# tensorlayer/HyperPose

Hardware: AMD Instinct MI355X
Metric: end-to-end FPS (preproc+DNN+PAF parse) @ 368x432 (higher is better)
Workload: dtype f32; 1 GPU; configs[1]: Lightweight-OpenPose (MobilenetDilated) + PAF parser, batch 8 @ 368x432 per GPU; frames from pinned host memory (one H2D per batch), parser on the network's own maps, humans to the host; key=configs[1]/f32, global_batch=8, parallelism=frame-sharded x1, no steady-state collective, pipes_per_gpu=4, parser_input=the network's own heat-maps

## Files before the change

### hyperpose_amd/csrc/conv_fp32.hip

```cpp
#include "conv_fp32.hpp"

#include "conv32_epilogue.hpp"
#include "conv_device.hpp"

#include <algorithm>
#include <cstdlib>

namespace hp {

namespace {

typedef float f32x4 __attribute__((ext_vector_type(4)));

__device__ __forceinline__ float act32(float v, int act, float param, float alpha)
{
    switch (act) {
    case ACT_RELU:
        return fmaxf(v, 0.f);
    case ACT_RELU6:
        return fminf(fmaxf(v, 0.f), 6.f);
    case ACT_LEAKY:
        return v > 0.f ? v : v * param;
    case ACT_PRELU:
        return v > 0.f ? v : v * alpha;
    case ACT_SIGMOID:
        return 1.f / (1.f + expf(-v));
    case ACT_SOFTPLUS:
        return v > 20.f ? v : log1pf(expf(v));
    default:
        return v;
    }
}

__device__ __forceinline__ long tv32_off(const tview32& t, int b, int y, int x)
{
    return ((long)b * t.img + (long)y * t.wp + x) * t.cs + t.coff;
}

}

template <int BM, int BN, int WM, int WN, bool ROWS>
__global__ __launch_bounds__(256) void conv32_kernel(const conv32_params p)
{
    constexpr int BK = 16, LDR = 20;
    constexpr int TM = BM / WM / 32, TN = BN / WN / 32, NA = BM / 64, NB = BN / 64;
    static_assert(WM * WN == 4 && TM >= 1 && TN >= 1 && NA >= 1 && NB >= 1, "tile");
    constexpr int AB_BYTES = 2 * (BM + BN) * LDR * 4, SLABS = 4 * rows_geom<TM>::SLAB_BYTES;
    __shared__ __attribute__((aligned(16))) unsigned char lds_raw[AB_BYTES > SLABS ? AB_BYTES : SLABS];
    float (*const sA)[BM * LDR] = reinterpret_cast<float (*)[BM * LDR]>(lds_raw);
    float (*const sB)[BN * LDR] = reinterpret_cast<float (*)[BN * LDR]>(lds_raw + 2 * BM * LDR * 4);

    const int tid = threadIdx.x, lane = tid & 63, wave = tid >> 6;
    const int wm = wave / WN, wn = wave % WN;
    const int G = p.Cout_pad / BM, nx = (p.npix + BN - 1) / BN;
    const int bj = blockIdx.x >> 3, ptile = (bj / G) * 8 + (blockIdx.x & 7);
    if (ptile >= nx)
        return;
    const int n0 = ptile * BN, m0 = (bj % G) * BM;
    const int lrow = tid >> 2, lchunk = (tid & 3) * 4;
    const int OHW = p.OH * p.OW, kc = p.Cin / BK, steps = p.KH * p.KW * kc;

    long bbase[NB];
#pragma unroll
    for (int j = 0; j < NB; ++j) {
        const int n = min(n0 + lrow + 64 * j, p.npix - 1);
        const int b = n / OHW, rem = n - b * OHW;
        const int oy = rem / p.OW, ox = rem - oy * p.OW;
        bbase[j] = tv32_off(p.in, b, oy * p.stride - p.pad_t, ox * p.stride - p.pad_l) + lchunk;
    }
    const float* const wrow = p.w + (long)(m0 + lrow) * p.Cin + lchunk;

    f32x4 ra[NA], rb[NB];
    auto gload = [&](int s) {
        const int tap = s / kc, k0 = (s - tap * kc) * BK;
        const int ky = tap / p.KW, kx = tap - ky * p.KW;
        const long toff = ((long)(ky * p.dil) * p.in.wp + kx * p.dil) * p.in.cs + k0;
        const float* const wt = wrow + (long)tap * p.Cout_pad * p.Cin + k0;
#pragma unroll
        for (int j = 0; j < NA; ++j)
            ra[j] = *reinterpret_cast<const f32x4*>(wt + (long)(64 * j) * p.Cin);
#pragma unroll
        for (int j = 0; j < NB; ++j)
            rb[j] = *reinterpret_cast<const f32x4*>(p.in.p + bbase[j] + toff);
    };
    auto to_lds = [&](int buf) {
#pragma unroll
        for (int j = 0; j < NA; ++j)
            *reinterpret_cast<f32x4*>(&sA[buf][(lrow + 64 * j) * LDR + lchunk]) = ra[j];
#pragma unroll
        for (int j = 0; j < NB; ++j)
            *reinterpret_cast<f32x4*>(&sB[buf][(lrow + 64 * j) * LDR + lchunk]) = rb[j];
    };

    floatx16 acc[TM][TN];
#pragma unroll
    for (int i = 0; i < TM; ++i)
#pragma unroll
        for (int j = 0; j < TN; ++j)
#pragma unroll
            for (int r = 0; r < 16; ++r)
                acc[i][j][r] = 0.f;

    const int frow = lane & 31, fh = (lane >> 5) * 4;
    int dbg_i = 0;
#define HP_STAMP()                                       \
    if (p.dbg && blockIdx.x == 9 && tid == 0)            \
        p.dbg[dbg_i++] = __builtin_amdgcn_s_memtime();
    HP_STAMP();
    if (p.dbg && tid == 0 && blockIdx.x < 4096) {
        p.dbg[128 + 3 * blockIdx.x] = __builtin_amdgcn_s_memrealtime();
        p.dbg[128 + 3 * blockIdx.x + 2] = ((unsigned long long)__builtin_amdgcn_s_getreg((31 << 11) | 20) << 32) | (unsigned)__builtin_amdgcn_s_getreg((31 << 11) | 4);
    }
    gload(0);
    to_lds(0);
    lds_barrier();
    HP_STAMP();
#pragma unroll 1
    for (int s = 0; s < steps; ++s) {
        gload(min(s + 1, steps - 1));
        const float* const a_s = &sA[s & 1][(wm * TM * 32 + frow) * LDR + fh];
        const float* const b_s = &sB[s & 1][(wn * TN * 32 + frow) * LDR + fh];
#pragma unroll
        for (int kk = 0; kk < BK / 8; ++kk) {
            f32x4 fa[TM], fb[TN];
#pragma unroll
            for (int i = 0; i < TM; ++i)
                fa[i] = *reinterpret_cast<const f32x4*>(a_s + i * 32 * LDR + kk * 8);
#pragma unroll
            for (int j = 0; j < TN; ++j)
                fb[j] = *reinterpret_cast<const f32x4*>(b_s + j * 32 * LDR + kk * 8);
#pragma unroll
            for (int e = 0; e < 4; ++e)
#pragma unroll
                for (int i = 0; i < TM; ++i)
#pragma unroll
                    for (int j = 0; j < TN; ++j)
                        acc[i][j] = __builtin_amdgcn_mfma_f32_32x32x2f32(fa[i][e], fb[j][e], acc[i][j], 0, 0, 0);
        }
        to_lds((s + 1) & 1);
        lds_barrier();
        if ((s & 7) == 7)
            HP_STAMP();
    }

    if constexpr (ROWS) {
        lds_barrier();
        float* const slab = reinterpret_cast<float*>(lds_raw) + wave * (rows_geom<TM>::SLAB_BYTES / 4);
#pragma unroll
        for (int j = 0; j < TN; ++j) {
            floatx16 fin[TM];
#pragma unroll
            for (int i = 0; i < TM; ++i)
                fin[i] = acc[i][j];
            const int nb = n0 + (wn * TN + j) * 32;
            conv32_store_rows<TM>(p, fin, slab, lane, m0 + wm * TM * 32, [&](int r, bool& ok, long& ooff, long& roff) {
                const int n = nb + r;
                ok = n < p.npix;
                const int nc = min(n, p.npix - 1);
                const int b = nc / OHW, rem = nc - b * OHW;
                const int oy = rem / p.OW, ox = rem - oy * p.OW;
                ooff = tv32_off(p.out, b, oy, ox);
                roff = p.res.p ? tv32_off(p.res, b, oy, ox) : 0;
            });
        }
    } else {
    const bool out_vec = p.out.p && ((p.out.coff | p.out.cs) & 3) == 0;
    const bool res_vec = p.res.p && ((p.res.coff | p.res.cs) & 3) == 0;
    const bool res_pre = p.res.p && p.res_before_act, res_post = p.res.p && !p.res_before_act;
#pragma unroll
    for (int j = 0; j < TN; ++j) {
        const int n = n0 + (wn * TN + j) * 32 + frow;
        const bool pix_ok = n < p.npix;
        const int nc = min(n, p.npix - 1);
        const int b = nc / OHW, rem = nc - b * OHW;
        const int oy = rem / p.OW, ox = rem - oy * p.OW;
        const long ooff = p.out.p ? tv32_off(p.out, b, oy, ox) : 0;
        const long roff = p.res.p ? tv32_off(p.res, b, oy, ox) : 0;
#pragma unroll
        for (int i = 0; i < TM; ++i) {
#pragma unroll
            for (int q = 0; q < 4; ++q) {
                const int m = m0 + (wm * TM + i) * 32 + 8 * q + fh;
                if (pix_ok && m < p.Cout) {
                    const bool full = m + 3 < p.Cout;
                    float v[4], rr[4] = { 0.f, 0.f, 0.f, 0.f };
                    if (p.res.p) {
                        if (full && res_vec) {
                            const f32x4 t = *reinterpret_cast<const f32x4*>(p.res.p + roff + m);
                            rr[0] = t[0], rr[1] = t[1], rr[2] = t[2], rr[3] = t[3];
                        } else {
#pragma unroll
                            for (int e = 0; e < 4; ++e)
                                if (m + e < p.Cout)
                                    rr[e] = p.res.p[roff + m + e];
                        }
                    }
                    const f32x4 bs = *reinterpret_cast<const f32x4*>(p.bias + m);
                    f32x4 sl = { p.act_slope, p.act_slope, p.act_slope, p.act_slope };
                    if (p.alpha)
                        sl = *reinterpret_cast<const f32x4*>(p.alpha + m);
#pragma unroll
                    for (int e = 0; e < 4; ++e) {
                        float x = acc[i][j][4 * q + e] + bs[e];
                        if (res_pre)
                            x += rr[e];
                        x = x > 0.f ? fminf(x, p.act_hi) : x * sl[e];
                        if (res_post)
                            x += rr[e];
                        v[e] = x;
                    }
                    if (p.out.p) {
                        if (full && out_vec) {
                            f32x4 t = { v[0], v[1], v[2], v[3] };
                            *reinterpret_cast<f32x4*>(p.out.p + ooff + m) = t;
                        } else {
#pragma unroll
                            for (int e = 0; e < 4; ++e)
                                if (m + e < p.Cout)
                                    p.out.p[ooff + m + e] = v[e];
                        }
                    }
                    if (p.out_f32) {
#pragma unroll
                        for (int e = 0; e < 4; ++e)
                            if (m + e < p.Cout)
                                p.out_f32[((long)b * p.Cout + m + e) * OHW + rem] = v[e];
                    }
                }
            }
        }
    }
    }
    HP_STAMP();
    if (p.dbg && tid == 0 && blockIdx.x < 4096)
        p.dbg[128 + 3 * blockIdx.x + 1] = __builtin_amdgcn_s_memrealtime();
#undef HP_STAMP
}

template <int BN, int WN = 2>
__global__ __launch_bounds__(256) void conv32_t16_kernel(const conv32_params p)
{
    constexpr int BM = 64, BK = 16, WM = 4 / WN, TMW = BM / 16 / WM, TNW = BN / WN / 16;
    constexpr int NB = (BN + 63) / 64, BR = NB * 64;
    static_assert(BN % (16 * WN) == 0 && (WN == 1 || WN == 2), "wavefront columns of whole 16-pixel tiles");
    __shared__ __attribute__((aligned(16))) float lds[2 * (BM + BR) * BK];
    float (*const sA)[BM * BK] = reinterpret_cast<float (*)[BM * BK]>(lds);
    float (*const sB)[BR * BK] = reinterpret_cast<float (*)[BR * BK]>(lds + 2 * BM * BK);

    const int tid = threadIdx.x, lane = tid & 63, wave = tid >> 6;
    const int wm = WN == 2 ? wave >> 1 : wave, wn = WN == 2 ? wave & 1 : 0;
    const int G = p.Cout_pad / BM, nx = (p.npix + BN - 1) / BN;
    const int bj = blockIdx.x >> 3, ptile = (bj / G) * 8 + (blockIdx.x & 7);
    if (ptile >= nx)
        return;
    const int n0 = ptile * BN, m0 = (bj % G) * BM;
    const int lrow = tid >> 2, lq = tid & 3;
    const int OHW = p.OH * p.OW, kc = p.Cin / BK, steps = p.KH * p.KW * kc;
    auto swz = [](int row, int quad) { return row * BK + ((quad ^ (((row >> 3) & 1) << 1)) << 2); };

    long bbase[NB];
#pragma unroll
    for (int j = 0; j < NB; ++j) {
        const int n = min(n0 + min(lrow + 64 * j, BN - 1), p.npix - 1);
        const int b = n / OHW, rem = n - b * OHW;
        const int oy = rem / p.OW, ox = rem - oy * p.OW;
        bbase[j] = tv32_off(p.in, b, oy * p.stride - p.pad_t, ox * p.stride - p.pad_l) + lq * 4;
    }
    const float* const wrow = p.w + (long)(m0 + lrow) * p.Cin + lq * 4;
    f32x4 ra, rb[NB];
    auto gload = [&](int s) {
        const int tap = s / kc, k0 = (s - tap * kc) * BK;
        const int ky = tap / p.KW, kx = tap - ky * p.KW;
        const long toff = ((long)(ky * p.dil) * p.in.wp + kx * p.dil) * p.in.cs + k0;
        ra = *reinterpret_cast<const f32x4*>(wrow + (long)tap * p.Cout_pad * p.Cin + k0);
#pragma unroll
        for (int j = 0; j < NB; ++j)
            rb[j] = *reinterpret_cast<const f32x4*>(p.in.p + bbase[j] + toff);
    };
    auto to_lds = [&](int buf) {
        *reinterpret_cast<f32x4*>(&sA[buf][swz(lrow, lq)]) = ra;
#pragma unroll
        for (int j = 0; j < NB; ++j)
            *reinterpret_cast<f32x4*>(&sB[buf][swz(lrow + 64 * j, lq)]) = rb[j];
    };

    f32x4 acc[TMW][TNW];
#pragma unroll
    for (int i = 0; i < TMW; ++i)
#pragma unroll
        for (int j = 0; j < TNW; ++j)
            acc[i][j] = f32x4{ 0.f, 0.f, 0.f, 0.f };

    const int fr = lane & 15, kq = lane >> 4;
    int dbg_i = 0;
#define HP_STAMP()                                       \
    if (p.dbg && blockIdx.x == 9 && tid == 0)            \
        p.dbg[dbg_i++] = __builtin_amdgcn_s_memtime();
    HP_STAMP();
    if (p.dbg && tid == 0 && blockIdx.x < 4096) {
        p.dbg[128 + 3 * blockIdx.x] = __builtin_amdgcn_s_memrealtime();
        p.dbg[128 + 3 * blockIdx.x + 2] = ((unsigned long long)__builtin_amdgcn_s_getreg((31 << 11) | 20) << 32) | (unsigned)__builtin_amdgcn_s_getreg((31 << 11) | 4);
    }
    gload(0);
    to_lds(0);
    lds_barrier();
    HP_STAMP();
#pragma unroll 1
    for (int s = 0; s < steps; ++s) {
        gload(min(s + 1, steps - 1));
        f32x4 fa[TMW], fb[TNW];
#pragma unroll
        for (int i = 0; i < TMW; ++i)
            fa[i] = *reinterpret_cast<const f32x4*>(&sA[s & 1][swz(wm * (16 * TMW) + i * 16 + fr, kq)]);
#pragma unroll
        for (int j = 0; j < TNW; ++j)
            fb[j] = *reinterpret_cast<const f32x4*>(&sB[s & 1][swz(wn * (BN / WN) + j * 16 + fr, kq)]);
#pragma unroll
        for (int e = 0; e < 4; ++e)
#pragma unroll
            for (int i = 0; i < TMW; ++i)
#pragma unroll
                for (int j = 0; j < TNW; ++j)
                    acc[i][j] = __builtin_amdgcn_mfma_f32_16x16x4f32(fa[i][e], fb[j][e], acc[i][j], 0, 0, 0);
        to_lds((s + 1) & 1);
        lds_barrier();
        if ((s & 7) == 7)
            HP_STAMP();
    }

    const int q = lane >> 4;
    const bool out_vec = p.out.p && ((p.out.coff | p.out.cs) & 3) == 0;
    const bool res_vec = p.res.p && ((p.res.coff | p.res.cs) & 3) == 0;
    const bool res_pre = p.res.p && p.res_before_act, res_post = p.res.p && !p.res_before_act;
    f32x4 bs[TMW], sl[TMW];
#pragma unroll
    for (int i = 0; i < TMW; ++i) {
        const int m = m0 + wm * (16 * TMW) + i * 16 + 4 * q;
        bs[i] = *reinterpret_cast<const f32x4*>(p.bias + m);
        sl[i] = f32x4{ p.act_slope, p.act_slope, p.act_slope, p.act_slope };
        if (p.alpha)
            sl[i] = *reinterpret_cast<const f32x4*>(p.alpha + m);
    }
#pragma unroll
    for (int j = 0; j < TNW; ++j) {
        const int n = n0 + wn * (BN / WN) + j * 16 + fr;
        const bool pix_ok = n < p.npix;
        const int nc = min(n, p.npix - 1);
        const int b = nc / OHW, rem = nc - b * OHW;
        const int oy = rem / p.OW, ox = rem - oy * p.OW;
        const long ooff = p.out.p ? tv32_off(p.out, b, oy, ox) : 0;
        const long roff = p.res.p ? tv32_off(p.res, b, oy, ox) : 0;
#pragma unroll
        for (int i = 0; i < TMW; ++i) {
            const int m = m0 + wm * (16 * TMW) + i * 16 + 4 * q;
            if (!pix_ok || m >= p.Cout)
                continue;
            const bool full = m + 3 < p.Cout;
            float v[4], rr[4] = { 0.f, 0.f, 0.f, 0.f };
            if (p.res.p) {
                if (full && res_vec) {
                    const f32x4 t = *reinterpret_cast<const f32x4*>(p.res.p + roff + m);
                    rr[0] = t[0], rr[1] = t[1], rr[2] = t[2], rr[3] = t[3];
                } else {
#pragma unroll
                    for (int e = 0; e < 4; ++e)
                        if (m + e < p.Cout)
                            rr[e] = p.res.p[roff + m + e];
                }
            }
#pragma unroll
            for (int e = 0; e < 4; ++e) {
                float x = acc[i][j][e] + bs[i][e];
                if (res_pre)
                    x += rr[e];
                x = x > 0.f ? fminf(x, p.act_hi) : x * sl[i][e];
                if (res_post)
                    x += rr[e];
                v[e] = x;
            }
            if (p.out.p) {
                if (full && out_vec)
                    *reinterpret_cast<f32x4*>(p.out.p + ooff + m) = f32x4{ v[0], v[1], v[2], v[3] };
                else {
#pragma unroll
                    for (int e = 0; e < 4; ++e)
                        if (m + e < p.Cout)
                            p.out.p[ooff + m + e] = v[e];
                }
            }
// ... 131 lines not shown
                const long ooff = s_out[prow] + m;
                float v[4], rv[4] = { 0.f, 0.f, 0.f, 0.f };
                if (p.res.p) {
                    if (res_vec) {
                        rv[0] = rr[j][h][r][0], rv[1] = rr[j][h][r][1], rv[2] = rr[j][h][r][2], rv[3] = rr[j][h][r][3];
                    } else {
                        const long roff = s_res[prow] + m;
#pragma unroll
                        for (int e = 0; e < 4; ++e)
                            if (m + e < p.Cout)
                                rv[e] = p.res.p[roff + e];
                    }
                }
#pragma unroll
                for (int e = 0; e < 4; ++e) {
                    float x = a[e] + bsr[h][e];
                    if (res_pre)
                        x += rv[e];
                    x = x > 0.f ? fminf(x, p.act_hi) : x * slr[h][e];
                    if (res_post)
                        x += rv[e];
                    v[e] = x;
                }
                if (full && out_vec)
                    *reinterpret_cast<f32x4*>(p.out.p + ooff) = f32x4{ v[0], v[1], v[2], v[3] };
                else {
#pragma unroll
                    for (int e = 0; e < 4; ++e)
                        if (m + e < p.Cout)
                            p.out.p[ooff + e] = v[e];
                }
            }
            __builtin_amdgcn_wave_barrier();
        }
    }
}

template <int KT, int BN>
static hipError_t launch_wk(const conv32_params& p, dim3 grid, hipStream_t s)
{
    constexpr int lds = KT / 16 * ((64 * 16 + 16) + (BN * 16 + 16)) * 4 + 4 * 16 * 36 * 4 + 3 * BN * 8;
    static bool granted = false;
    if (lds > 64 * 1024 && !granted) {
        const hipError_t e = hipFuncSetAttribute((const void*)conv32_wk_kernel<KT, BN>, hipFuncAttributeMaxDynamicSharedMemorySize, lds);
        if (e != hipSuccess)
            return e;
        granted = true;
    }
    HP_LAUNCH((conv32_wk_kernel<KT, BN>), grid, dim3(256), lds, s, p);
    return hipGetLastError();
}

static int conv32_wk_bn(const conv32_params& p, const engine_switches& sw)
{
    const int wk = sw.c32_wk;
    if (wk == 0 || p.KH != 1 || p.KW != 1 || p.dil != 1 || p.out_f32 || !p.out.p || (p.Cin != 32 && p.Cin != 64 && p.Cin != 128))
        return 0;
    if (p.Cin == 128 && wk != 1)
        return 0;
    const int bn = 64;
    const long np = p.pick_npix > 0 ? p.pick_npix : p.npix, blocks = (np + bn - 1) / bn * (p.Cout_pad / 64);
    return wk == 1 || blocks >= 768 ? bn : 0;
}

static void conv32_pick(const conv32_params& p, const engine_switches& sw, int& BM, int& BN)
{
    BM = p.Cout_pad % 128 == 0 ? 128 : 64, BN = 128;
    const long blocks = (long)(((p.pick_npix > 0 ? p.pick_npix : p.npix) + 127) / 128) * (p.Cout_pad / BM);
    if (blocks < 448)
        BM = 64, BN = 64;
    else if (blocks < 1024 && BM == 128)
        BM = 64;
    const int bn160 = sw.c32_bn160;
    if (bn160 == 1 || bn160 == 176) {
        BM = 64, BN = bn160 == 1 ? 160 : 176;
        return;
    }
    if (BM == 64 && BN == 128 && bn160 != 0) {
        const long np = p.pick_npix > 0 ? p.pick_npix : p.npix;
        const long g = p.Cout_pad / 64, b128 = (long)((np + 127) / 128) * g, b160 = (long)((np + 159) / 160) * g;
        if (b128 > 1024 && b160 <= 1024)
            BN = 160;
    }
    if (bn160 != 0 && p.KH == 1 && p.KW == 1 && p.stride == 1 && p.Cin <= 128 && p.Cout_pad >= 256 && !p.out_f32 && (BN == 128))
        BM = 64, BN = 160;
}

static bool conv32_rows(const conv32_params& p, int BN)
{
    if (BN == 160 || BN == 176)
        return false;
    return !p.out_f32 && (p.lane_epilogue < 0 || (p.lane_epilogue == 0 && BN == 64));
}

int conv32_tile(const conv32_params& p, const engine_switches& sw)
{
    if (const int bn = conv32_wk_bn(p, sw))
        return 39000000 + p.Cin * 1000 + bn;
    int BM, BN;
    conv32_pick(p, sw, BM, BN);
    return 32000000 + (conv32_rows(p, BN) ? 400000 : 0) + BM * 1000 + BN;
}

bool set_act32(conv32_params& p)
{
    const float inf = __builtin_huge_valf();
    switch (p.act) {
    case ACT_NONE:
        p.act_slope = 1.f, p.act_hi = inf;
        return true;
    case ACT_RELU:
        p.act_slope = 0.f, p.act_hi = inf;
        return true;
    case ACT_RELU6:
        p.act_slope = 0.f, p.act_hi = 6.f;
        return true;
    case ACT_LEAKY:
        p.act_slope = p.act_param, p.act_hi = inf;
        return true;
    case ACT_PRELU:
        p.act_slope = 0.f, p.act_hi = inf;
        return p.alpha != nullptr;
    default:
        return false;
    }
}

hipError_t launch_conv32(const conv32_params& p, const engine_switches& sw, hipStream_t s)
{
    if (p.Cin % 16 || p.Cout_pad % 64 || p.npix <= 0)
        return hipErrorInvalidValue;
    if (const int bn = conv32_wk_bn(p, sw)) {
        const dim3 g(((p.npix + bn - 1) / bn + 7) / 8 * 8 * (p.Cout_pad / 64));
        return p.Cin == 32 ? launch_wk<32, 64>(p, g, s) : p.Cin == 64 ? launch_wk<64, 64>(p, g, s) : launch_wk<128, 64>(p, g, s);
    }
    int BM, BN;
    conv32_pick(p, sw, BM, BN);
    const dim3 grid(((p.npix + BN - 1) / BN + 7) / 8 * 8 * (p.Cout_pad / BM));
    const bool rows = conv32_rows(p, BN);
#define HP_C32_CASE(BM_, BN_, WM_, WN_)                                                    \
    if (rows)                                                                              \
        HP_LAUNCH((conv32_kernel<BM_, BN_, WM_, WN_, true>), grid, dim3(256), 0, s, p);    \
    else                                                                                   \
        HP_LAUNCH((conv32_kernel<BM_, BN_, WM_, WN_, false>), grid, dim3(256), 0, s, p);
    if (BN == 176) {
        HP_LAUNCH((conv32_t16_kernel<176, 1>), grid, dim3(256), 0, s, p);
    } else if (BN == 160) {
        HP_LAUNCH((conv32_t16_kernel<160>), grid, dim3(256), 0, s, p);
    } else if (BM == 128) {
        HP_C32_CASE(128, 128, 2, 2)
    } else if (BN == 128) {
        HP_C32_CASE(64, 128, 1, 4)
    } else {
        HP_C32_CASE(64, 64, 2, 2)
    }
#undef HP_C32_CASE
    return hipGetLastError();
}

__device__ unsigned g_first_conv_verify[4];
__global__ __launch_bounds__(256) void first_conv32_kernel(const first_conv32_params p, int tiles_x, int tiles_y, int TH, int GP, int verify)
{
    extern __shared__ __attribute__((aligned(16))) float s_w32[];
    constexpr int TW = 8, PX = 4;
    const int G = (p.Cout + 7) / 8, CP = G * 8, taps = p.KH * p.KW;
    const int IH = (TH - 1) * p.stride + p.KH, IW = (TW - 1) * p.stride + p.KW;
    float* const s_x = s_w32 + taps * 3 * CP;
    int t = blockIdx.x;
    const int tx = t % tiles_x;
    t /= tiles_x;
    const int ty = t % tiles_y, b = t / tiles_y;
    const int oy0 = ty * TH, ox0 = tx * TW;
    const int iy0 = oy0 * p.stride - p.pad_t, ix0 = ox0 * p.stride - p.pad_l;
    for (int i = threadIdx.x; i < taps * 3 * CP; i += 256) {
        const int co = i % CP, tc = i / CP;
        s_w32[i] = co < p.Cout ? p.w[(size_t)co * taps * 3 + tc] : 0.f;
    }
    for (int i = threadIdx.x; i < IH * IW; i += 256) {
        const int py = i / IW, px = i - py * IW;
        const int iy = iy0 + py, ix = ix0 + px;
        float v[3] = { 0.f, 0.f, 0.f };
        if (iy >= 0 && iy < p.H && ix >= 0 && ix < p.W) {
            if (p.in_u8) {
                const uint8_t* q = p.in_u8 + (((size_t)b * p.H + iy) * p.W + ix) * 3;
#pragma unroll
                for (int c = 0; c < 3; ++c)
                    v[c] = ((float)((double)q[p.flip_rb ? 2 - c : c] * p.factor) - p.mean[c]) * p.inv_std[c];
            } else {
#pragma unroll
                for (int c = 0; c < 3; ++c)
                    v[c] = (p.in_f32[(((size_t)b * 3 + c) * p.H + iy) * p.W + ix] - p.mean[c]) * p.inv_std[c];
            }
        }
        s_x[i * 3] = v[0], s_x[i * 3 + 1] = v[1], s_x[i * 3 + 2] = v[2];
    }
    __syncthreads();
    const int g0 = threadIdx.x % GP, slot = threadIdx.x / GP;
    auto verify_lds = [&]() {
        if (!verify)
            return;
        unsigned bad_x = 0, bad_w = 0;
        for (int i = threadIdx.x; i < IH * IW; i += 256) {
            const int py = i / IW, px = i - py * IW;
            const int iy = iy0 + py, ix = ix0 + px;
            float v[3] = { 0.f, 0.f, 0.f };
            if (iy >= 0 && iy < p.H && ix >= 0 && ix < p.W && p.in_u8) {
                const uint8_t* q = p.in_u8 + (((size_t)b * p.H + iy) * p.W + ix) * 3;
                for (int c = 0; c < 3; ++c)
                    v[c] = ((float)((double)q[p.flip_rb ? 2 - c : c] * p.factor) - p.mean[c]) * p.inv_std[c];
            }
            for (int c = 0; c < 3; ++c)
                bad_x += __float_as_uint(s_x[i * 3 + c]) != __float_as_uint(v[c]);
        }
        for (int i = threadIdx.x; i < taps * 3 * CP; i += 256) {
            const int co = i % CP, tc = i / CP;
            const float wv = co < p.Cout ? p.w[(size_t)co * taps * 3 + tc] : 0.f;
            bad_w += __float_as_uint(s_w32[i]) != __float_as_uint(wv);
        }
        if (bad_x)
            atomicAdd(&g_first_conv_verify[0], bad_x);
        if (bad_w)
            atomicAdd(&g_first_conv_verify[1], bad_w);
        if (threadIdx.x == 0)
            atomicAdd(&g_first_conv_verify[2], 1u);
    };
    if (slot >= TH * (TW / PX)) {
        verify_lds();
        return;
    }
    const int ly = slot / (TW / PX), lx0 = (slot % (TW / PX)) * PX;
    const int oy = oy0 + ly;
    if (oy >= p.OH) {
        verify_lds();
        return;
    }
    const bool vec_ok = ((p.out.coff | p.out.cs) & 3) == 0;
    for (int g = g0; g < G; g += GP) {
        float acc[PX][8];
#pragma unroll
        for (int r = 0; r < 8; ++r) {
            const float bv = (g * 8 + r < p.Cout) ? p.bias[g * 8 + r] : 0.f;
#pragma unroll
            for (int j = 0; j < PX; ++j)
                acc[j][r] = bv;
        }
        for (int ky = 0; ky < p.KH; ++ky)
            for (int kx = 0; kx < p.KW; ++kx) {
                const float* xp = s_x + ((ly * p.stride + ky) * IW + lx0 * p.stride + kx) * 3;
                const float* wt = s_w32 + (size_t)((ky * p.KW + kx) * 3) * CP + g * 8;
#pragma unroll
                for (int c = 0; c < 3; ++c) {
                    const f32x4 w0 = *reinterpret_cast<const f32x4*>(wt + c * CP);
                    const f32x4 w1 = *reinterpret_cast<const f32x4*>(wt + c * CP + 4);
#pragma unroll
                    for (int j = 0; j < PX; ++j) {
                        const float xv = xp[j * p.stride * 3 + c];
#pragma unroll
                        for (int e = 0; e < 4; ++e)
                            acc[j][e] = fmaf(xv, w0[e], acc[j][e]), acc[j][4 + e] = fmaf(xv, w1[e], acc[j][4 + e]);
                    }
                }
            }
        if (verify) {
            float acc2[PX][8];
#pragma unroll
            for (int r = 0; r < 8; ++r) {
                const float bv = (g * 8 + r < p.Cout) ? p.bias[g * 8 + r] : 0.f;
#pragma unroll
                for (int j = 0; j < PX; ++j)
                    acc2[j][r] = bv;
            }
            for (int ky = 0; ky < p.KH; ++ky)
                for (int kx = 0; kx < p.KW; ++kx) {
                    const float* xp = s_x + ((ly * p.stride + ky) * IW + lx0 * p.stride + kx) * 3;
                    const float* wt = s_w32 + (size_t)((ky * p.KW + kx) * 3) * CP + g * 8;
#pragma unroll
                    for (int c = 0; c < 3; ++c) {
                        const f32x4 w0 = *reinterpret_cast<const f32x4*>(wt + c * CP);
                        const f32x4 w1 = *reinterpret_cast<const f32x4*>(wt + c * CP + 4);
#pragma unroll
                        for (int j = 0; j < PX; ++j) {
                            const float xv = xp[j * p.stride * 3 + c];
#pragma unroll
                            for (int e = 0; e < 4; ++e)
                                acc2[j][e] = fmaf(xv, w0[e], acc2[j][e]), acc2[j][4 + e] = fmaf(xv, w1[e], acc2[j][4 + e]);
                        }
                    }
                }
            unsigned bad = 0;
#pragma unroll
            for (int j = 0; j < PX; ++j)
#pragma unroll
                for (int r = 0; r < 8; ++r)
                    bad += __float_as_uint(acc[j][r]) != __float_as_uint(acc2[j][r]);
            if (bad)
                atomicAdd(&g_first_conv_verify[3], bad);
        }
#pragma unroll
        for (int j = 0; j < PX; ++j) {
            const int ox = ox0 + lx0 + j;
            if (ox >= p.OW)
                break;
            float* op = p.out.p + tv32_off(p.out, b, oy, ox) + g * 8;
            if (g * 8 + 7 < p.Cout && vec_ok) {
                f32x4 o0, o1;
#pragma unroll
                for (int e = 0; e < 4; ++e)
// ... 293 lines not shown
```

### hyperpose_amd/csrc/engine.cpp

```cpp
#include "conv_fp32.hpp"
#include "conv_i8.hpp"
#include "conv_kernels.hpp"
#include "engine_timeline.hpp"
#include "hp_common.hpp"
#include "weight_pack.hpp"

#include <algorithm>
#include <cmath>
#include <map>
#include <memory>
#include <string>
#include <variant>
#include <cstdio>
#include <cstdlib>
#include <vector>

namespace {

inline int round_up(int a, int b) { return (a + b - 1) / b * b; }

struct tensor_info {
    bool defined = false;
    bool elided = false;
    bool unwritten = false;
// ... 1654 lines not shown
{
    hd = hp::timeline_header{};
    hd.layer = st.layer;
    switch (st.kind) {
    case launch_kind::conv16: {
        const auto& c = std::get<conv16_launch>(b);
        if (c.i8 || !switches.dbg_conv || hp::conv_mfma_tile(c.cp) / 100000 != 52)
            return false;
        kind = hp::timeline_kind::conv, hd.cin = c.cp.Cin, hd.cout = c.cp.Cout, hd.tile = hp::conv_mfma_tile(c.cp);
        return true;
    }
    case launch_kind::bneck:
        kind = hp::timeline_kind::bneck, hd.tile = hp::bottleneck_variant(std::get<hp::bneck_params>(b));
        return switches.dbg_bn;
    case launch_kind::chain:
        kind = hp::timeline_kind::chain, hd.tile = hp::conv_chain_variant(std::get<hp::chain_params>(b));
        return switches.dbg_chain;
    case launch_kind::sep:
        kind = hp::timeline_kind::sep, hd.cin = std::get<hp::sep_params>(b).C;
        return switches.dbg_sep;
    case launch_kind::conv32:
    case launch_kind::wino2:
    case launch_kind::wino3:
    case launch_kind::direct: {
        const hp::conv32_params& q = std::get<conv32_launch>(b).cp;
        if (!switches.dbg_direct || (st.kind == launch_kind::conv32 && q.Cin < switches.dbg_min_cin))
            return false;
        kind = st.kind == launch_kind::conv32 ? hp::timeline_kind::conv32
            : st.kind == launch_kind::wino2   ? hp::timeline_kind::wino
            : st.kind == launch_kind::wino3   ? hp::timeline_kind::wino3
                                              : hp::timeline_kind::direct;
        hd.cin = q.Cin, hd.cout = q.Cout, hd.kh = q.KH, hd.kw = q.KW, hd.tile = tile_of(st.kind, b);
        if (st.kind == launch_kind::wino2)
            (void)hp::conv32_winograd_occupancy(q, &hd.blocks_per_cu);
        return true;
    }
    default: return false;
    }
}

int hp_engine::trace_step(const step& st, launch_payload& b, hipStream_t s) const
{
    hp::timeline_kind kind;
    hp::timeline_header hd;
    if (!timeline_of(st, b, kind, hd))
        return HP_OK;
    const size_t words = hp::timeline_words(kind);
    hp::dev_buf buf;
    HP_TRY(buf.alloc(words * 8));
    HP_HIP_TRY(hipMemset(buf.p, 0, words * 8));
    HP_TRY(launch(st.kind, b, s, buf.as<unsigned long long>()));
    HP_HIP_TRY(hipStreamSynchronize(s));
    std::vector<unsigned long long> hv(words);
    HP_HIP_TRY(hipMemcpy(hv.data(), buf.p, words * 8, hipMemcpyDeviceToHost));
    hp::print_timeline(stderr, kind, hd, hv.data());
    return HP_OK;
}

int hp_engine::run_step(const step& st, const uint8_t* u8, const float* f32, int n, hipStream_t s, int b0) const
{
    launch_payload b = bound(st, u8, f32, n, b0);
    HP_TRY(launch(st.kind, b, s, nullptr));
    return trace_step(st, b, s);
}

int hp_engine::launch_head_pair32(size_t i, int n, int b0, hipStream_t s, bool* done) const
{
    *done = false;
    if (i + 1 >= steps.size() || steps[i].kind != launch_kind::head32 || steps[i + 1].kind != launch_kind::head32)
        return HP_OK;
    const auto &ha = steps[i].as<head32_launch>(), &hb = steps[i + 1].as<head32_launch>();
    const hp::conv32_params a = bind(ha.cp, n, b0), b = bind(hb.cp, n, b0);
    if (!hp::conv32_head_pair_ok(a, b, switches))
        return HP_OK;
    HP_HIP_TRY(hp::launch_conv32_head_pair(a, ha.hh, b, hb.hh, s));
    *done = true;
    return HP_OK;
}

int hp_engine::enqueue_range(const uint8_t* u8, const float* f32, int b0, int n, hipStream_t s) const
{
    for (size_t i = 0; i < steps.size(); ++i) {
        bool paired = false;
        HP_TRY(launch_head_pair32(i, n, b0, s, &paired));
        if (paired)
            ++i;
        else
            HP_TRY(run_step(steps[i], u8, f32, n, s, b0));
    }
    for (auto& o : outputs)
        if (o.fused_layer < 0) {
            const tensor_info& ti = *tensors[o.tensor];
            float* const dst = o.buf->as<float>() + (size_t)b0 * o.out_c() * o.x.out_h * o.x.out_w;
            if (is_f32())
                HP_HIP_TRY(hp::launch_output_transform32(at_frame(ti.view32(o.coff), b0), n, o.H, o.W, o.x, dst, s));
            else
                HP_HIP_TRY(hp::launch_output_transform(ti.view(o.coff), n, o.H, o.W, o.x, dst, s));
        }
    return HP_OK;
}

void hp_engine::fill_row(hp_layer_time* out, int k, int cap, const step& st, int n, float ms) const
{
    if (!out || k >= cap)
        return;
    out[k].layer = st.layer, out[k].op = st.op;
    out[k].tile = step_tile(st, n);
    out[k].ms = ms;
    out[k].flops = st.flops * n, out[k].bytes = st.bytes * n;
}

int hp_engine::stage_profile_input()
{
    const size_t need = (size_t)max_batch * in_h * in_w * 3 * sizeof(float);
    if (in_stage.bytes < need)
        HP_TRY(in_stage.alloc(need));
    return HP_OK;
}

int hp_engine::enqueue(const uint8_t* u8, const float* f32, int n, hipStream_t s, const void* host_src, size_t frame_bytes) const
{
    unsigned char* const dev_in = u8 ? (unsigned char*)u8 : (unsigned char*)f32;
    auto h2d = [&](int b0, int cnt, hipStream_t st) -> int {
        if (host_src)
            HP_HIP_TRY(hipMemcpyAsync(dev_in + (size_t)b0 * frame_bytes, (const unsigned char*)host_src + (size_t)b0 * frame_bytes, (size_t)cnt * frame_bytes, hipMemcpyHostToDevice, st));
        return HP_OK;
    };
    if (parts < 2 || !halves_ok() || n < 2) {
        HP_TRY(h2d(0, n, s));
        return enqueue_range(u8, f32, 0, n, s);
    }
    const int n0 = (n + 1) / 2;
    HP_HIP_TRY(hipEventRecord(ev_fork, s));
    HP_HIP_TRY(hipStreamWaitEvent(stream2, ev_fork, 0));
    HP_TRY(h2d(0, n0, s));
    HP_TRY(h2d(n0, n - n0, stream2));
    HP_TRY(enqueue_range(u8, f32, 0, n0, s));
    HP_TRY(enqueue_range(u8, f32, n0, n - n0, stream2));
    HP_HIP_TRY(hipEventRecord(ev_join, stream2));
    HP_HIP_TRY(hipStreamWaitEvent(s, ev_join, 0));
    return HP_OK;
}

hp::engine_switches hp::read_engine_switches()
{
    auto on = [](const char* name) { return getenv(name) != nullptr; };
    auto num = [](const char* name, int unset) { const char* v = getenv(name); return v ? atoi(v) : unset; };
    engine_switches w;
    w.no_fuse = on("HP_NO_FUSE"), w.no_fuse_head = num("HP_NO_FUSE_HEAD", 0) != 0, w.no_splitk = on("HP_NO_SPLITK");
    w.no_chain = on("HP_NO_CHAIN"), w.no_bneck = on("HP_NO_BNECK"), w.no_seppair = on("HP_NO_SEPPAIR"), w.no_pair_heads = on("HP_NO_PAIR_HEADS");
    w.fuse32 = on("HP_FUSE32"), w.no_fuse32 = on("HP_NO_FUSE32"), w.no_head32 = on("HP_NO_HEAD32"), w.no_arena = on("HP_NO_ARENA");
    w.no_winograd32 = on("HP_NO_WINOGRAD32"), w.wino_f33 = num("HP_WINO_F33", 0) == 1, w.wino_tall = num("HP_WINO_TALL", 1) != 0;
    w.wino_nc = num("HP_WINO_NC", 0), w.head_pair32 = num("HP_HEAD_PAIR", 1) != 0;
    w.c32_wk = num("HP_C32_WK", -1), w.c32_bn160 = num("HP_C32_BN160", -1), w.dw32_px = num("HP_DW32_PX", 0);
    w.lane_epilogue = num("HP_LANE_EPILOGUE", 0), w.first_conv_verify = on("HP_FIRST_CONV_VERIFY");
    w.dbg_conv = on("HP_CONV_DBG"), w.dbg_bn = on("HP_BN_DBG"), w.dbg_chain = on("HP_CHAIN_DBG"), w.dbg_sep = on("HP_SEP_DBG");
    w.dbg_direct = on("HP_DIRECT_DBG"), w.dbg_min_cin = num("HP_DIRECT_DBG_MINCIN", 256);
    return w;
}

extern "C" {

int hp_engine_create(hp_engine** out, const hp_engine_desc* desc)
{
    HP_REQUIRE(out && desc, HP_ERR_INVALID, "hp_engine_create: null argument");
    std::unique_ptr<hp_engine> e(new hp_engine());
    e->switches = hp::read_engine_switches();
    try {
        HP_TRY(e->build(desc));
    } catch (const std::exception& ex) {
        HP_REQUIRE(false, HP_ERR_INVALID, "hp_engine_create: %s", ex.what());
    }
    *out = e.release();
    return HP_OK;
}

namespace {
constexpr char ENGINE_MAGIC[8] = { 'H', 'P', 'E', 'N', 'G', '0', '0', '3' };
struct engine_file_header {
    char magic[8];
    int32_t layer_size, output_size;
    int32_t in_w, in_h, max_batch, flip_rb;
    double factor;
    float mean[3], inv_std[3];
    int32_t n_layers, n_outputs;
    uint64_t n_weights;
    int32_t dtype;
    int32_t n_scales;
};
}

int hp_engine_save(const hp_engine* e, const char* path)
{
    HP_REQUIRE(e && path, HP_ERR_INVALID, "hp_engine_save: null argument");
    FILE* f = fopen(path, "wb");
    HP_REQUIRE(f, HP_ERR_INVALID, "hp_engine_save: cannot open %s for writing", path);
    engine_file_header h{};
    memcpy(h.magic, ENGINE_MAGIC, 8);
    h.layer_size = (int32_t)sizeof(hp_layer), h.output_size = (int32_t)sizeof(hp_output_desc);
    h.in_w = e->in_w, h.in_h = e->in_h, h.max_batch = e->max_batch, h.flip_rb = e->flip_rb, h.factor = e->factor;
    for (int c = 0; c < 3; ++c)
        h.mean[c] = e->mean[c], h.inv_std[c] = e->inv_std[c];
    h.n_layers = (int32_t)e->layers.size(), h.n_outputs = (int32_t)e->out_descs.size(), h.n_weights = e->weights_blob.size();
    h.dtype = e->dtype;
    h.n_scales = (int32_t)e->i8_scale.size();
    bool ok = fwrite(&h, sizeof(h), 1, f) == 1;
    ok = ok && fwrite(e->layers.data(), sizeof(hp_layer), e->layers.size(), f) == e->layers.size();
    ok = ok && fwrite(e->out_descs.data(), sizeof(hp_output_desc), e->out_descs.size(), f) == e->out_descs.size();
    ok = ok && fwrite(e->weights_blob.data(), sizeof(float), e->weights_blob.size(), f) == e->weights_blob.size();
    ok = ok && fwrite(e->i8_scale.data(), sizeof(float), e->i8_scale.size(), f) == e->i8_scale.size();
    ok = (fclose(f) == 0) && ok;
    HP_REQUIRE(ok, HP_ERR_INVALID, "hp_engine_save: short write to %s", path);
    return HP_OK;
}

int hp_engine_load(hp_engine** out, const char* path, int max_batch)
{
    HP_REQUIRE(out && path, HP_ERR_INVALID, "hp_engine_load: null argument");
    FILE* f = fopen(path, "rb");
    HP_REQUIRE(f, HP_ERR_INVALID, "hp_engine_load: cannot open %s", path);
    engine_file_header h{};
    std::vector<hp_layer> layers;
    std::vector<hp_output_desc> outs;
    std::vector<float> w, scales;
    constexpr size_t HDR_001 = offsetof(engine_file_header, dtype);
    bool ok = fread(&h, HDR_001, 1, f) == 1;
    if (ok && memcmp(h.magic, "HPENG001", 8) == 0)
        memcpy(h.magic, ENGINE_MAGIC, 8), h.dtype = HP_DTYPE_F16, h.n_scales = 0;
    else {
        ok = ok && fread(reinterpret_cast<char*>(&h) + HDR_001, sizeof(h) - HDR_001, 1, f) == 1;
        if (ok && memcmp(h.magic, "HPENG002", 8) == 0)
            memcpy(h.magic, ENGINE_MAGIC, 8), ok = h.n_scales == 0 && h.dtype != HP_DTYPE_I8;
    }
    ok = ok && memcmp(h.magic, ENGINE_MAGIC, 8) == 0 && h.layer_size == (int32_t)sizeof(hp_layer)
        && h.output_size == (int32_t)sizeof(hp_output_desc) && h.n_layers > 0 && h.n_layers < (1 << 20) && h.n_outputs > 0
        && h.n_outputs < 4096 && h.n_weights < ((uint64_t)1 << 34)
        && (h.dtype == HP_DTYPE_F16 || h.dtype == HP_DTYPE_F32 || h.dtype == HP_DTYPE_F32S || h.dtype == HP_DTYPE_I8)
        && h.n_scales == (h.dtype == HP_DTYPE_I8 ? h.n_layers : 0);
    if (ok) {
        const long at = ftell(f);
        ok = fseek(f, 0, SEEK_END) == 0;
        const long size = ftell(f);
        ok = ok && fseek(f, at, SEEK_SET) == 0
            && (uint64_t)size == (uint64_t)at + (uint64_t)h.n_layers * sizeof(hp_layer) + (uint64_t)h.n_outputs * sizeof(hp_output_desc) + h.n_weights * sizeof(float)
                    + (uint64_t)h.n_scales * sizeof(float);
    }
    if (ok) {
        layers.resize(h.n_layers), outs.resize(h.n_outputs), w.resize(h.n_weights), scales.resize(h.n_scales);
        ok = fread(layers.data(), sizeof(hp_layer), layers.size(), f) == layers.size()
            && fread(outs.data(), sizeof(hp_output_desc), outs.size(), f) == outs.size() && fread(w.data(), sizeof(float), w.size(), f) == w.size()
            && fread(scales.data(), sizeof(float), scales.size(), f) == scales.size();
    }
    fclose(f);
    HP_REQUIRE(ok, HP_ERR_INVALID, "hp_engine_load: %s is not an engine file written by this library version", path);
    hp_engine_desc d{};
    d.in_w = h.in_w, d.in_h = h.in_h, d.max_batch = max_batch > 0 ? max_batch : h.max_batch, d.factor = h.factor, d.flip_rb = h.flip_rb;
    for (int c = 0; c < 3; ++c)
        d.mean[c] = h.mean[c], d.inv_std[c] = h.inv_std[c];
    d.layers = layers.data(), d.n_layers = h.n_layers, d.outputs = outs.data(), d.n_outputs = h.n_outputs, d.weights = w.data(), d.n_weights = w.size();
    d.dtype = h.dtype;
    d.int8_scales = scales.empty() ? nullptr : scales.data();
    return hp_engine_create(out, &d);
}

void hp_engine_destroy(hp_engine* e)
{
    if (!e)
        return;
    if (e->stream)
        (void)hipStreamSynchronize(e->stream);
    delete e;
}

int hp_engine_max_batch(const hp_engine* e) { return e ? e->max_batch : HP_ERR_INVALID; }

int hp_engine_describe(const hp_engine* e, hp_engine_desc* d)
{
    HP_REQUIRE(e && d, HP_ERR_INVALID, "hp_engine_describe: null argument");
    d->in_w = e->in_w, d->in_h = e->in_h, d->max_batch = e->max_batch, d->factor = e->factor, d->flip_rb = e->flip_rb;
    for (int c = 0; c < 3; ++c)
        d->mean[c] = e->mean[c], d->inv_std[c] = e->inv_std[c];
    d->layers = e->layers.data(), d->n_layers = (int32_t)e->layers.size();
    d->outputs = e->out_descs.data(), d->n_outputs = (int32_t)e->out_descs.size();
    d->weights = e->weights_blob.data(), d->n_weights = e->weights_blob.size();
    d->dtype = e->dtype;
    d->int8_scales = e->dtype == HP_DTYPE_I8 ? e->i8_scale.data() : nullptr;
    return HP_OK;
}

int hp_engine_dtype(const hp_engine* e) { return e ? e->dtype : HP_ERR_INVALID; }

int hp_engine_input_size(const hp_engine* e, int* w, int* h)
{
    HP_REQUIRE(e && w && h, HP_ERR_INVALID, "hp_engine_input_size: null argument");
    *w = e->in_w, *h = e->in_h;
    return HP_OK;
}

int hp_engine::leave_split()
{
    HP_TRY(drop_graphs());
    split_off = true, ++split_fallbacks;
    *static_cast<volatile unsigned*>(ovf_flag.p) = 0;
    return HP_OK;
}

static int infer_common(hp_engine* e, const void* input, size_t frame_bytes, int n, int on_device, void* stream, int kind)
// ... 496 lines not shown
```

### hyperpose_amd/csrc/hp_common.hpp

```cpp
#pragma once
#include <hip/hip_runtime.h>

#include <cstdarg>
#include <cstdio>
#include <cstring>
#include <string>
#include <vector>

#include "../../include/hp_hip.h"

namespace hp {

void set_error(const char* fmt, ...) __attribute__((format(printf, 1, 2)));
const char* last_error();

#define HP_HIP_TRY(expr)                                                                                     \
    do {                                                                                                     \
        hipError_t _e = (expr);                                                                              \
        if (_e != hipSuccess) {                                                                              \
            ::hp::set_error("%s failed: %s (%s:%d)", #expr, hipGetErrorString(_e), __FILE__, __LINE__);      \
            return HP_ERR_HIP;                                                                               \
        }                                                                                                    \
    } while (0)

#define HP_REQUIRE(cond, code, ...)                                                                          \
    do {                                                                                                     \
        if (!(cond)) {                                                                                       \
            ::hp::set_error(__VA_ARGS__);                                                                    \
            return (code);                                                                                   \
        }                                                                                                    \
    } while (0)

#define HP_TRY(expr)                                                                                         \
    do {                                                                                                     \
        int _rc = (expr);                                                                                    \
        if (_rc != HP_OK)                                                                                    \
            return _rc;                                                                                      \
    } while (0)

struct dev_buf {
    void* p = nullptr;
    size_t bytes = 0;
    dev_buf() = default;
    dev_buf(const dev_buf&) = delete;
    dev_buf& operator=(const dev_buf&) = delete;
    ~dev_buf() { release(); }
    int alloc(size_t n)
    {
        release();
        if (n == 0)
            return HP_OK;
        HP_HIP_TRY(hipMalloc(&p, n));
        bytes = n;
        return HP_OK;
    }
    void release()
    {
        if (p)
            (void)hipFree(p);
        p = nullptr;
        bytes = 0;
    }
    template <typename T>
    T* as() const { return static_cast<T*>(p); }
};

struct host_buf {
    void* p = nullptr;
    size_t bytes = 0;
    host_buf() = default;
    host_buf(const host_buf&) = delete;
    host_buf& operator=(const host_buf&) = delete;
    ~host_buf() { release(); }
    int alloc(size_t n)
    {
        release();
        if (n == 0)
            return HP_OK;
        HP_HIP_TRY(hipHostMalloc(&p, n, hipHostMallocDefault));
        bytes = n;
        return HP_OK;
    }
    void release()
    {
        if (p)
            (void)hipHostFree(p);
        p = nullptr;
        bytes = 0;
    }
    template <typename T>
    T* as() const { return static_cast<T*>(p); }
};

inline int ceil_div(int a, int b) { return (a + b - 1) / b; }

int merge_humans(const hp_human* in, const int32_t* region_of, int n, int frame_w, int frame_h, int min_common, double tol, std::vector<hp_human>& kept);

struct engine_switches {
    bool no_fuse = false;
    bool no_fuse_head = false;
    bool no_splitk = false;
    bool no_chain = false;
    bool no_bneck = false;
    bool no_seppair = false;
    bool no_pair_heads = false;
    bool fuse32 = false;
    bool no_fuse32 = false;
    bool no_head32 = false;
    bool no_arena = false;
    bool no_winograd32 = false;
    bool wino_f33 = false;
    bool wino_tall = true;
    int wino_nc = 0;
    bool head_pair32 = true;
    int c32_wk = -1;
    int c32_bn160 = -1;
    int dw32_px = 0;
    int lane_epilogue = 0;
    bool first_conv_verify = false;
    bool dbg_conv = false, dbg_bn = false, dbg_chain = false, dbg_sep = false;
    bool dbg_direct = false;
    int dbg_min_cin = 256;
};
engine_switches read_engine_switches();

class frame_pool {
public:
    static frame_pool& instance();
    int workers() const { return n_threads_ + 1; }
    void run(int n_frames, void (*fn)(int frame, int worker, void* ctx), void* ctx);
    ~frame_pool();

private:
    frame_pool();
    struct impl;
    impl* d_;
    int n_threads_;
};

}
```

Measured before the change: 5382 frames/s.

## Deepen global-load prefetch in 64x64 fp32 conv kernel to two stages

Refactors the fp32 implicit-GEMM conv kernel into a body templated on prefetch depth D, holding D sets of register staging buffers so global loads for step s+D are issued while step s computes. The 64x64 tile variant defaults to depth 2, and an environment switch selects depth 1 or 3. The aim is to hide more global-memory latency behind the MFMA work. In exchange it uses more VGPRs for staging, which can reduce occupancy, and the loop is unrolled by U.

New measurement: 5423 frames/s, median of 6. Within noise of the previous version (+0.8%).

```diff
diff --git a/hyperpose_amd/csrc/conv_fp32.hip b/hyperpose_amd/csrc/conv_fp32.hip
--- a/hyperpose_amd/csrc/conv_fp32.hip
+++ b/hyperpose_amd/csrc/conv_fp32.hip
@@ -39,10 +39,11 @@
 
 }
 
-template <int BM, int BN, int WM, int WN, bool ROWS>
-__global__ __launch_bounds__(256) void conv32_kernel(const conv32_params p)
+template <int BM, int BN, int WM, int WN, bool ROWS, int D>
+__device__ __forceinline__ void conv32_body(const conv32_params p)
 {
     constexpr int BK = 16, LDR = 20;
+    static_assert(D >= 1 && D <= 3, "prefetch depth");
     constexpr int TM = BM / WM / 32, TN = BN / WN / 32, NA = BM / 64, NB = BN / 64;
     static_assert(WM * WN == 4 && TM >= 1 && TN >= 1 && NA >= 1 && NB >= 1, "tile");
     constexpr int AB_BYTES = 2 * (BM + BN) * LDR * 4, SLABS = 4 * rows_geom<TM>::SLAB_BYTES;
@@ -70,26 +71,26 @@
     }
     const float* const wrow = p.w + (long)(m0 + lrow) * p.Cin + lchunk;
 
-    f32x4 ra[NA], rb[NB];
-    auto gload = [&](int s) {
+    f32x4 ra[D][NA], rb[D][NB];
+    auto gload = [&](int d, int s) {
         const int tap = s / kc, k0 = (s - tap * kc) * BK;
         const int ky = tap / p.KW, kx = tap - ky * p.KW;
         const long toff = ((long)(ky * p.dil) * p.in.wp + kx * p.dil) * p.in.cs + k0;
         const float* const wt = wrow + (long)tap * p.Cout_pad * p.Cin + k0;
 #pragma unroll
         for (int j = 0; j < NA; ++j)
-            ra[j] = *reinterpret_cast<const f32x4*>(wt + (long)(64 * j) * p.Cin);
+            ra[d][j] = *reinterpret_cast<const f32x4*>(wt + (long)(64 * j) * p.Cin);
 #pragma unroll
         for (int j = 0; j < NB; ++j)
-            rb[j] = *reinterpret_cast<const f32x4*>(p.in.p + bbase[j] + toff);
+            rb[d][j] = *reinterpret_cast<const f32x4*>(p.in.p + bbase[j] + toff);
     };
-    auto to_lds = [&](int buf) {
+    auto to_lds = [&](int d, int buf) {
 #pragma unroll
         for (int j = 0; j < NA; ++j)
-            *reinterpret_cast<f32x4*>(&sA[buf][(lrow + 64 * j) * LDR + lchunk]) = ra[j];
+            *reinterpret_cast<f32x4*>(&sA[buf][(lrow + 64 * j) * LDR + lchunk]) = ra[d][j];
 #pragma unroll
         for (int j = 0; j < NB; ++j)
-            *reinterpret_cast<f32x4*>(&sB[buf][(lrow + 64 * j) * LDR + lchunk]) = rb[j];
+            *reinterpret_cast<f32x4*>(&sB[buf][(lrow + 64 * j) * LDR + lchunk]) = rb[d][j];
     };
 
     floatx16 acc[TM][TN];
@@ -111,15 +112,16 @@
         p.dbg[128 + 3 * blockIdx.x] = __builtin_amdgcn_s_memrealtime();
         p.dbg[128 + 3 * blockIdx.x + 2] = ((unsigned long long)__builtin_amdgcn_s_getreg((31 << 11) | 20) << 32) | (unsigned)__builtin_amdgcn_s_getreg((31 << 11) | 4);
     }
-    gload(0);
-    to_lds(0);
+#pragma unroll
+    for (int d = 0; d < D; ++d)
+        gload(d, min(d, steps - 1));
+    to_lds(0, 0);
     lds_barrier();
     HP_STAMP();
-#pragma unroll 1
-    for (int s = 0; s < steps; ++s) {
-        gload(min(s + 1, steps - 1));
-        const float* const a_s = &sA[s & 1][(wm * TM * 32 + frow) * LDR + fh];
-        const float* const b_s = &sB[s & 1][(wn * TN * 32 + frow) * LDR + fh];
+    auto kstep = [&](int u, int buf, int s) {
+        gload(u, min(s + D, steps - 1));
+        const float* const a_s = &sA[buf][(wm * TM * 32 + frow) * LDR + fh];
+        const float* const b_s = &sB[buf][(wn * TN * 32 + frow) * LDR + fh];
 #pragma unroll
         for (int kk = 0; kk < BK / 8; ++kk) {
             f32x4 fa[TM], fb[TN];
@@ -137,11 +139,23 @@
                     for (int j = 0; j < TN; ++j)
                         acc[i][j] = __builtin_amdgcn_mfma_f32_32x32x2f32(fa[i][e], fb[j][e], acc[i][j], 0, 0, 0);
         }
-        to_lds((s + 1) & 1);
+        to_lds((u + 1) % D, buf ^ 1);
         lds_barrier();
         if ((s & 7) == 7)
             HP_STAMP();
-    }
+    };
+    constexpr int U = D > 1 && D % 2 ? 2 * D : D;
+    int s = 0;
+#pragma unroll 1
+    for (; s + U <= steps; s += U) {
+#pragma unroll
+        for (int u = 0; u < U; ++u)
+            kstep(u % D, U % 2 ? s & 1 : u & 1, s + u);
+    }
+#pragma unroll
+    for (int u = 0; u < U - 1; ++u)
+        if (s + u < steps)
+            kstep(u % D, u & 1, s + u);
 
     if constexpr (ROWS) {
         lds_barrier();
@@ -235,6 +249,22 @@
     if (p.dbg && tid == 0 && blockIdx.x < 4096)
         p.dbg[128 + 3 * blockIdx.x + 1] = __builtin_amdgcn_s_memrealtime();
 #undef HP_STAMP
+}
+
+constexpr int C32_PF_64 = 2, C32_PF_MAX = 3;
+template <int BM, int BN>
+constexpr int conv32_depth = BM == 64 && BN == 64 ? C32_PF_64 : 1;
+
+template <int BM, int BN, int WM, int WN, bool ROWS>
+__global__ __launch_bounds__(256) void conv32_kernel(const conv32_params p)
+{
+    conv32_body<BM, BN, WM, WN, ROWS, conv32_depth<BM, BN>>(p);
+}
+
+template <int BM, int BN, int WM, int WN, bool ROWS, int D>
+__global__ __launch_bounds__(256) void conv32_pf_kernel(const conv32_params p)
+{
+    conv32_body<BM, BN, WM, WN, ROWS, D>(p);
 }
 
 template <int BN, int WN = 2>
@@ -672,7 +702,21 @@
     } else if (BN == 128) {
         HP_C32_CASE(64, 128, 1, 4)
     } else {
-        HP_C32_CASE(64, 64, 2, 2)
+        const int d = sw.c32_pf <= 0 ? C32_PF_64 : std::min(sw.c32_pf, C32_PF_MAX);
+#define HP_C32_PF_CASE(D_)                                                                   \
+    if (rows)                                                                                \
+        HP_LAUNCH((conv32_pf_kernel<64, 64, 2, 2, true, D_>), grid, dim3(256), 0, s, p);     \
+    else                                                                                     \
+        HP_LAUNCH((conv32_pf_kernel<64, 64, 2, 2, false, D_>), grid, dim3(256), 0, s, p);
+        static_assert(C32_PF_64 == 2 && C32_PF_MAX == 3, "the depths beside the rule's");
+        if (d == C32_PF_64) {
+            HP_C32_CASE(64, 64, 2, 2)
+        } else if (d == 1) {
+            HP_C32_PF_CASE(1)
+        } else {
+            HP_C32_PF_CASE(3)
+        }
+#undef HP_C32_PF_CASE
     }
 #undef HP_C32_CASE
     return hipGetLastError();
diff --git a/hyperpose_amd/csrc/engine.cpp b/hyperpose_amd/csrc/engine.cpp
--- a/hyperpose_amd/csrc/engine.cpp
+++ b/hyperpose_amd/csrc/engine.cpp
@@ -1830,7 +1830,7 @@
     w.fuse32 = on("HP_FUSE32"), w.no_fuse32 = on("HP_NO_FUSE32"), w.no_head32 = on("HP_NO_HEAD32"), w.no_arena = on("HP_NO_ARENA");
     w.no_winograd32 = on("HP_NO_WINOGRAD32"), w.wino_f33 = num("HP_WINO_F33", 0) == 1, w.wino_tall = num("HP_WINO_TALL", 1) != 0;
     w.wino_nc = num("HP_WINO_NC", 0), w.head_pair32 = num("HP_HEAD_PAIR", 1) != 0;
-    w.c32_wk = num("HP_C32_WK", -1), w.c32_bn160 = num("HP_C32_BN160", -1), w.dw32_px = num("HP_DW32_PX", 0);
+    w.c32_wk = num("HP_C32_WK", -1), w.c32_bn160 = num("HP_C32_BN160", -1), w.c32_pf = num("HP_C32_PF", 0), w.dw32_px = num("HP_DW32_PX", 0);
     w.lane_epilogue = num("HP_LANE_EPILOGUE", 0), w.first_conv_verify = on("HP_FIRST_CONV_VERIFY");
     w.dbg_conv = on("HP_CONV_DBG"), w.dbg_bn = on("HP_BN_DBG"), w.dbg_chain = on("HP_CHAIN_DBG"), w.dbg_sep = on("HP_SEP_DBG");
     w.dbg_direct = on("HP_DIRECT_DBG"), w.dbg_min_cin = num("HP_DIRECT_DBG_MINCIN", 256);
diff --git a/hyperpose_amd/csrc/hp_common.hpp b/hyperpose_amd/csrc/hp_common.hpp
--- a/hyperpose_amd/csrc/hp_common.hpp
+++ b/hyperpose_amd/csrc/hp_common.hpp
@@ -115,6 +115,7 @@
     bool head_pair32 = true;
     int c32_wk = -1;
     int c32_bn160 = -1;
+    int c32_pf = 0;
     int dw32_px = 0;
     int lane_epilogue = 0;
     bool first_conv_verify = false;
```
